# rcleuthold/awebox

Hardware: AMD Instinct MI355X
Metric: NLP f/g/Jacobian evals/sec, AP2 N=40 d=4 (higher is better)
Workload: dtype f64; 1 GPU; AP2 single kite, direct collocation radau N=40 d=4 zoh, 2048 NLP instances per step and GPU, one eval = f + g + grad f + J_g; n_v=6154, n_g=6103, nnz_jac=84726, batch_per_gpu=2048, parallelism=replicas x1

## Files before the change

### awebox_amd/csrc/awegpu.hip

```cpp
#include <hip/hip_runtime.h>

#include <algorithm>
#include <cmath>
#include <cstdio>
#include <cstdlib>
#include <cstring>
#include <memory>
#include <string>
#include <vector>

#include "../../include/awegpu.h"
#include "../../include/awegpu_rk4root.h"
#include "host_util.hpp"
#include "ap2_model.hpp"
#ifndef AWE_GEN_HEADER
#define AWE_GEN_HEADER "ap2_nodejac.gen.hpp"
#endif
#include AWE_GEN_HEADER
#include "ap2_tables.hpp"
#include "im_layout.hpp"

namespace {

using namespace awt;
using namespace hostu;




struct KArgs {
    const double* V;
    const double* P;
    const double* cst;
    DevColl coll;
    const ColorTabs* ct;
    const int* seg;
    const unsigned* glist;
    const int* glist_off;
    double* g;
    double* jac;
    double* grad;
    double* partial;
    double* f;
    int n_k, d, n_v, n_g, n_p, nnz, batch;
    int stride, rows, v_int0;
    int tang_total;
    int nscale;
    double kconst[kMaxConst];
    int nconst;
    int want_derivs;
    const double* nodebuf;
    int nb_stride;
    size_t tan_shoot, tan_radau;
    const double* objb;
    int ld;
    int grad_ld;
    int in_ld;
};

struct LaneIn {
    const double* w;
    unsigned long long seedA;
    unsigned int seedXD;
    double cxx;
    double tfs;
    __device__ __forceinline__ static double bit(unsigned long long m, int i) {
        return (double)(unsigned)((m >> i) & 1ull);
    }
    __device__ __forceinline__ awe::Dual operator()(int i) const {
        double t = bit(seedA, i);
        if (i >= AWE_NX && i < 2 * AWE_NX) {
            const int j = i - AWE_NX;
            if ((seedA >> j) & 1ull) t += cxx;
            if ((seedXD >> j) & 1u) t += 1.0;
            t += tfs * w[i];
        }
        return awe::Dual(w[i], t);
    }
};

struct NodeSink {
    double* tp;
    double* gv;
    double* dump;
    unsigned long long cm;
    bool c0;
    __device__ __forceinline__ void emit(int r, const awe::Dual& v) {
        double* ga = c0 ? gv + r : dump;
        *ga = v.v;
        const bool on = (cm >> r) & 1ull;
        double* ta = on ? tp + __popcll(cm & ((1ull << r) - 1ull)) : dump;
        *ta = v.d;
    }
    __device__ __forceinline__ void eq_row(int r, const awe::Dual& v) { emit(r, v); }
    __device__ __forceinline__ void ineq_row(int r, const awe::Dual& v) { emit(AWE_N_EQ + r, v); }
    __device__ __forceinline__ void power(const awe::Dual& v) { emit(kRowPower, v); }
    __device__ __forceinline__ void beta(const awe::Dual& v) { emit(kRowBeta, v); }
};


constexpr int kPreDirs = 7;
__device__ __forceinline__ int pre_var(int j) { return j < 6 ? j : kDirDiam; }

struct LdsSubmodels {
    const double* pr;
    unsigned long long seedA;
    __device__ __forceinline__ void kite_atmosphere(const awe::Dual&, const double*, awe::Dual& uw,
                                                    awe::Dual& rho) const {
        const double sd = ((seedA >> 2) & 1ull) ? 1.0 : 0.0;
        uw = awe::Dual(pr[24], sd * pr[25]);
        rho = awe::Dual(pr[26], sd * pr[27]);
    }
    __device__ __forceinline__ void tether_drag(const awe::Dual*, const awe::Dual*, const awe::Dual&,
                                                const double*, const double*, awe::Dual D[3]) const {
#pragma unroll
        for (int i = 0; i < 3; ++i) {
            double t = 0.0;
#pragma unroll
            for (int j = 0; j < kPreDirs; ++j)
                if ((seedA >> pre_var(j)) & 1ull) t += pr[3 + 3 * j + i];
            D[i] = awe::Dual(pr[i], t);
        }
    }
};

__device__ __forceinline__ double wave_sum(double v) {
#pragma unroll
    for (int off = 32; off > 0; off >>= 1) v += __shfl_xor(v, off);
    return v;
}

template <int D>
constexpr int waves_for() { return (D + 2) / 2; }

template <int D>
constexpr int nloc_pad() {
    return ((9 + AWE_NX + AWE_NU + AWE_NX + AWE_NZ + D * (AWE_NX + AWE_NZ) + AWE_NX) + 1) & ~1;
}

constexpr int kPstCost = 64, kPstThRef = 84, kPstRef = 86;
template <int D>
constexpr int pst_pad() {
    return (kPstRef + AWE_NX + AWE_NU + AWE_NX + AWE_NZ + D * (AWE_NX + AWE_NZ) + 1) & ~1;
}

template <int D>
constexpr int lds_fixed_doubles() {
    return nloc_pad<D>() + pst_pad<D>() + (D + 1) * (64 + kGvalStride + 64 + kPreStride) + ((D + 2) & ~1) + 64 + 2;
}


template <int D, int NT>
__device__ __forceinline__ void node_values_pass(const double* vloc, const double* C, int n_k, double* wn,
                                                 int tid) {
    constexpr int NN = D + 1;
    const double* vt = vloc;
    const double* vx = vloc + 9;
    const double* vu = vx + AWE_NX;
    const double* vxd = vu + AWE_NU;
    const double* vz = vxd + AWE_NX;
    const double* vcoll = vz + AWE_NZ;
// ... 599 lines not shown
    for (int i = tid; i < a.nscale; i += NT) {
        double sv = 1.0;
        if (i >= 1 && i <= NN * NN) sv = C[i - 1] * inv_h_tf;
        else if (i > NN * NN) sv = a.kconst[i - 1 - NN * NN];
        scl[i] = sv;
    }
    node_values_pass<D, NT>(vloc, C, a.n_k, wn, tid);
    if (tid == 0) tl[a.tang_total] = 1.0;

    const double* pcost = pst + kPstCost;
    const double* pw8 = pst;
    const double psi = vt[2 + kPhiPsi];
    const double w_track = pcost[kCostTracking] / a.cst[AWE_C_NORM_TRACKING];
    const double w_xdot = pcost[kCostXdotRegularisation] / a.cst[AWE_C_NORM_XDOT_REG];
    const double w_ureg = pcost[kCostURegularisation] / a.cst[AWE_C_NORM_U_REG];
    const double w_fict = pcost[kCostFictitious] / a.cst[AWE_C_NORM_FICTITIOUS];
    const double w_theta = pcost[kCostThetaRegularisation] / a.cst[AWE_C_NORM_THETA_REG];
    for (int n = 1 + wave; n < NN; n += W) {
        const int dir = lane;
        const int j = n - 1;
        const double wj = a.coll.w[j];
        const double* w = wn + n * 64;
        const double* rb = pst + kPstRef;
        const double* rcx = rb + 2 * AWE_NX + AWE_NU + AWE_NZ + j * (AWE_NX + AWE_NZ);
        const double* ru = rb + AWE_NX;
        const double cxx = C[n * NN + n] * inv_h_tf;
        double trk = 0.0, xdr = 0.0, oth = 0.0, dfd = 0.0;
        if (dir < AWE_NX) {
            const double e = w[dir] - rcx[dir], ww = pw8[dir] * w_track;
            const double xdv = w[AWE_NX + dir], wx = pw8[AWE_NX + dir] * w_xdot;
            trk = ww * (e * e);
            dfd = wj * (psi * (2.0 * ww * e) + cxx * (2.0 * wx * xdv));
        } else if (dir < 2 * AWE_NX) {
            const double xdv = w[dir], wx = pw8[dir] * w_xdot;
            xdr = wx * (xdv * xdv);
            dfd = wj * (2.0 * wx * xdv);
        } else if (dir < 2 * AWE_NX + AWE_NU) {
            const int i = dir - 2 * AWE_NX;
            const double e = w[dir] - ru[i], wu = pw8[dir] * (i < 6 ? w_fict : w_ureg);
            oth = wu * (e * e);
            dfd = wj * (2.0 * wu * e);
        } else if (dir == kDirZ) {
            const double e = w[dir] - rcx[AWE_NX], ww = pw8[dir] * w_track;
            trk = ww * (e * e);
            dfd = wj * psi * (2.0 * ww * e);
        } else if (dir == kDirDiam) {
            const double e = w[dir] - pst[kPstThRef], wt = pw8[dir] * w_theta;
            oth = wt * (e * e);
            dfd = wj * (2.0 * wt * e);
        }
        trk = wave_sum(trk);
        xdr = wave_sum(xdr);
        oth = wave_sum(oth);
        const double* on = objn + j * kObjNode;
        const double bv = on[0], pv = on[1];
        const double cb = pcost[kCostBeta] * wj / a.cst[AWE_C_NORM_BETA];
        const double cp = -pcost[kCostPower] * wj / (double)a.n_k;
        if (dir == kDirTf) dfd = -2.0 * wj * xdr * inv_tf;
        if (dir == kDirPsi) dfd = wj * trk - cp * pv;
#pragma unroll
        for (int i = 0; i < awe_gen::kNDbp; ++i)
            if (dir == awe_gen::kDbpDir[i]) dfd += on[2 + i];
        dfl[n * 64 + dir] = dfd;
        if (dir == 0) fnode[n] = wj * (psi * trk + xdr + oth) + cb * (bv * bv) + (1.0 - psi) * (cp * pv);
    }
    __syncthreads();

    const DevColl* cc = &a.coll;
    for (int i = tid; i < AWE_NX; i += NT) {
        double xf = 0.0;
#pragma unroll
        for (int rr = 0; rr < NN; ++rr) {
            if (cc->D[rr] == 0.0) continue;
            const double Xr = (rr == 0) ? vx[i] : vcoll[(rr - 1) * (AWE_NX + AWE_NZ) + i];
            xf += cc->D[rr] * Xr;
        }
        g[k * a.rows + AWE_N_EQ + AWE_N_INEQ + D * AWE_N_EQ + i] = vx1[i] - xf;
    }
    double* part = a.partial + ((size_t)b * a.n_k + k) * kNPartial;
    if (tid == 0) {
        double s = 0.0;
        for (int n = 1; n < NN; ++n) s += fnode[n];
        part[0] = s;
    }
    if (tid >= 1 && tid <= 3) {
        const int dcol = tid == 1 ? kDirDiam : (tid == 2 ? kDirTf : kDirPsi);
        double s = 0.0;
        for (int n = 1; n < NN; ++n) s += dfl[n * 64 + dcol];
        part[tid] = s;
    }
    for (int col = tid; col < a.stride; col += NT) {
        double gsum = 0.0;
        if (col < AWE_NX) {
#pragma unroll
            for (int n = 1; n < NN; ++n) gsum += C[n] * inv_h_tf * dfl[n * 64 + AWE_NX + col];
        } else if (col < AWE_NX + AWE_NU) {
            const int i = col - AWE_NX;
#pragma unroll
            for (int n = 1; n < NN; ++n) gsum += dfl[n * 64 + 2 * AWE_NX + i];
        } else if (col >= 2 * AWE_NX + AWE_NU + AWE_NZ) {
            const int q = col - (2 * AWE_NX + AWE_NU + AWE_NZ);
            const int r = 1 + q / (AWE_NX + AWE_NZ), e = q % (AWE_NX + AWE_NZ);
            if (e < AWE_NX) {
                gsum = dfl[r * 64 + e];
#pragma unroll
                for (int n = 1; n < NN; ++n)
                    if (n != r) gsum += C[r * NN + n] * inv_h_tf * dfl[n * 64 + AWE_NX + e];
            } else {
                gsum = dfl[r * 64 + kDirZ];
            }
        }
        grad[base + col] = gsum;
    }
    int g0s[kSegs], los[kSegs];
#pragma unroll
    for (int q = 0; q < kSegs; ++q) { g0s[q] = sg[3 * q]; los[q] = sg[3 * q + 2]; }
#pragma unroll
    for (int u = 0; u < kGatherPerThread; ++u) {
        const int i = tid + u * NT;
        if (i < total) {
            int g0 = g0s[0], lo = los[0];
#pragma unroll
            for (int q = 1; q < kSegs; ++q)
                if (i >= los[q]) { g0 = g0s[q]; lo = los[q]; }
            jac[g0 + i - lo] = scl[ge[u] >> 16] * tl[ge[u] & 0xffffu];
        }
    }
}

constexpr int kSoaMinBatch = 128;

using SoaSlots = im::SlotTraits<awe_gen::kTanIdx, awe_gen::kNTan, AWE_NX, 512>;
inline bool soa_xdot_slot(int kind, int slot) {
    static const im::SlotTab<SoaSlots> st2(2);
    return kind == 1 && st2.cnt[1][slot] == 2;
}
template <int KIND>
struct SoaJSink1 {
    double* jac;
    unsigned lb;
    const unsigned* dt;
    const double* xs;
    struct Ref {
        const SoaJSink1* s;
        int slot;
        __device__ __forceinline__ void operator=(double v) const { s->put(slot, v); }
    };
    __device__ __forceinline__ Ref operator[](int slot) const { return Ref{this, slot}; }
    __device__ __forceinline__ void put(int slot, double v) const {
        const bool xd = KIND == 1 && im::kSlots<SoaSlots, 2>.cnt[1][slot] == 2;
        __builtin_nontemporal_store(xd ? xs[0] * v : v, &im::at_byte(jac, dt[im::kSlots<SoaSlots, 1>.first[KIND][slot]] + lb));
    }
};
template <int D, int KIND>
using SoaJSink = std::conditional_t<D == 1, SoaJSink1<KIND>, im::JSink<SoaSlots, D, KIND>>;

struct SoaNodeArgs {
    DevColl coll;
    int n_k, batch, ld, n_v, n_g, n_p, stride, v_int0, rows, nib, total, dstride;
    unsigned ldj8;
    unsigned gld8;
    double kconst[kMaxConst];
};

__global__ __launch_bounds__(256) void ap2_soa_in_kernel(const double* __restrict__ V, const double* __restrict__ P,
                                                         double* __restrict__ VT, double* __restrict__ PT,
                                                         int batch, int n_v, int n_p, int ld) {
    im::transpose_in<true>(V, P, VT, PT, batch, n_v, n_p, ld);
}

__global__ __launch_bounds__(256) void soa_to_aos_kernel(const double* __restrict__ src, size_t ld,
                                                         double* __restrict__ dst, int batch, int n) {
    __shared__ double tile[64][65];
    const int i0 = blockIdx.x * 64, b0 = blockIdx.y * 64;
    const int tid = threadIdx.x;
    double r[16];
#pragma unroll
    for (int it = 0; it < 16; ++it) {
        const int e = tid + it * 256, il = e >> 6, bl = e & 63;
        r[it] = src[(size_t)min(i0 + il, n - 1) * ld + min(b0 + bl, batch - 1)];
    }
#pragma unroll
    for (int it = 0; it < 16; ++it) {
        const int e = tid + it * 256;
        tile[e >> 6][e & 63] = r[it];
    }
    __syncthreads();
#pragma unroll
    for (int it = 0; it < 16; ++it) {
        const int e = tid + it * 256, bl = e >> 6, il = e & 63;
        if (i0 + il < n && b0 + bl < batch)
            __builtin_nontemporal_store(tile[il][bl], &dst[(size_t)(b0 + bl) * n + i0 + il]);
    }
}

__global__ __launch_bounds__(256) void aos_to_soa_kernel(const double* __restrict__ src, double* __restrict__ dst,
                                                         size_t ld, int batch, int n) {
    __shared__ double tile[64][65];
    const int i0 = blockIdx.x * 64, b0 = blockIdx.y * 64;
    const int tid = threadIdx.x;
    double r[16];
#pragma unroll
    for (int it = 0; it < 16; ++it) {
        const int e = tid + it * 256, bl = e >> 6, il = e & 63;
        r[it] = src[(size_t)min(b0 + bl, batch - 1) * n + min(i0 + il, n - 1)];
    }
#pragma unroll
    for (int it = 0; it < 16; ++it) {
        const int e = tid + it * 256;
        tile[e >> 6][e & 63] = r[it];
    }
    __syncthreads();
#pragma unroll
    for (int it = 0; it < 16; ++it) {
        const int e = tid + it * 256, il = e >> 6, bl = e & 63;
        if (i0 + il < n && b0 + bl < batch) dst[(size_t)(i0 + il) * ld + b0 + bl] = tile[bl][il];
    }
}

#ifndef AWE_SOA_WAVES_PER_EU
#define AWE_SOA_WAVES_PER_EU 1
#endif

constexpr int kSoaG = awe_gen::kNThUsed;
constexpr int kSoaGlob = 6;
constexpr int kSoaCO = 2 * AWE_NX + AWE_NU + AWE_NZ;
constexpr int kSoaShootWaves = 3;
template <int D>
constexpr int soa_radau_waves() { return D < 4 ? D : 4; }
template <int D>
constexpr int soa_radau_rows() { return kSoaG + kSoaGlob + kSoaCO + D * (AWE_NX + AWE_NZ); }
constexpr int soa_shoot_rows() { return kSoaG + kSoaGlob + kSoaShootWaves * kSoaCO; }

struct SoaThUsed {
    short idx[awe_gen::kNThUsed > 0 ? awe_gen::kNThUsed : 1];
    constexpr SoaThUsed() : idx() {
        for (int i = 0; i < AWE_NTHETA0; ++i)
            if (awe_gen::kThRow[i] >= 0) idx[awe_gen::kThRow[i]] = (short)i;
    }
};
constexpr SoaThUsed kSoaThUsed{};
constexpr bool soa_th_used_ok() {
    int named[awe_gen::kNThUsed > 0 ? awe_gen::kNThUsed : 1] = {};
    for (int i = 0; i < AWE_NTHETA0; ++i) {
        const int r = awe_gen::kThRow[i];
        if (r >= awe_gen::kNThUsed) return false;
        if (r >= 0) ++named[r];
    }
    for (int r = 0; r < awe_gen::kNThUsed; ++r) {
        const int i = kSoaThUsed.idx[r];
        if (named[r] != 1 || i < 0 || i >= AWE_NTHETA0 || awe_gen::kThRow[i] != r) return false;
    }
    return true;
}
static_assert(soa_th_used_ok(), "kSoaThUsed is not the inverse of kThRow over the rows [0, kSoaG)");

struct SoaLdsTh {
    const double* l;
    __device__ __forceinline__ double operator[](int i) const { return l[awe_gen::kThRow[i] * 64]; }
};

__device__ __forceinline__ unsigned soa_glob_src(int q, unsigned& which) {
    which = q < 4 ? 0u : 1u;
    return q == 0 ? 1u : q == 1 ? 0u : q == 2 ? (unsigned)(AWE_NTH + kPhiGamma)
         : q == 3 ? (unsigned)(AWE_NTH + kPhiPsi) : q == 4 ? (unsigned)kCostBeta : (unsigned)kCostPower;
}

template <int I>
struct SoaWaveC { static constexpr int value = I; };
template <int W, int WV = 0, class F>
__device__ __forceinline__ void soa_per_wave(int wave, const F& f) {
    if constexpr (WV + 1 < W) {
        if (wave != WV) return soa_per_wave<W, WV + 1>(wave, f);
    }
    f(SoaWaveC<WV>{});
}

template <int NT, int U>
struct SoaOffsetLoads {
    unsigned r[U];
    template <class Src>
    __device__ __forceinline__ void issue(int n, int tid, const Src& src) {
#pragma unroll
        for (int u = 0; u < U; ++u) r[u] = *src(tid + u * NT < n ? tid + u * NT : n - 1);
    }
    __device__ __forceinline__ void commit(unsigned* dst, int n, unsigned row8, int tid) const {
#pragma unroll
        for (int u = 0; u < U; ++u)
            if (tid + u * NT < n) dst[tid + u * NT] = r[u] * row8;
    }
};

template <int W, int NROWS, int NTAB, class RowOf, class TabSrc>
__device__ __forceinline__ void soa_stage(double* lds, unsigned* ldt, int tid, int wave, int ib, int nact,
                                          const double* VT, const double* THT, unsigned ld8, unsigned row8,
                                          const RowOf& row_of, const TabSrc& tab_src) {
    constexpr int NT = 64 * W, UT = (NTAB + NT - 1) / NT;
    const int lane = tid & 63;
    const unsigned lb = 8u * (unsigned)(ib * 64 + (lane < nact ? lane : 0));
    double* lw = lds + lane;
    soa_per_wave<W>(wave, [&](auto wc) {
        constexpr int WV = decltype(wc)::value;
        constexpr int J = (NROWS - WV + W - 1) / W;
        constexpr int NF = (J + UT + 62) / 63, F = (J + UT + NF - 1) / NF;
        static_assert(F <= 63 && J > (NF - 1) * F, "a flight of more loads than vmcnt counts");
        auto load = [&](int r) {
            unsigned which;
            const unsigned row = row_of(r, which);
            return im::at(which ? THT : VT, row, ld8, lb);
        };
        SoaOffsetLoads<NT, UT> tab;
#pragma unroll
        for (int f = 0; f < NF; ++f) {
            double v[F];
#pragma unroll
            for (int j = f * F; j < J && j < (f + 1) * F; ++j) v[j - f * F] = load(WV + j * W);
            if (f == NF - 1) tab.issue(NTAB, tid, tab_src);
#pragma unroll
            for (int j = f * F; j < J && j < (f + 1) * F; ++j) lw[(WV + j * W) * 64] = v[j - f * F];
        }
        tab.commit(ldt, NTAB, row8, tid);
    });
}

struct SoaLdsShootIn {
    const double* l;
    int base;
    __device__ __forceinline__ double at(int r) const { return l[r * 64]; }
    __device__ __forceinline__ double operator()(int i) const {
        if (i < AWE_NX) return at(base + i);
        if (i < 2 * AWE_NX) return at(base + AWE_NX + AWE_NU + (i - AWE_NX));
        if (i < 2 * AWE_NX + AWE_NU) return at(base + AWE_NX + (i - 2 * AWE_NX));
        if (i < 2 * AWE_NX + AWE_NU + AWE_NZ) return at(base + 2 * AWE_NX + AWE_NU);
        if (i < AWE_NW) return at(kSoaG + (i == 2 * AWE_NX + AWE_NU + AWE_NZ ? 1 : 0));
        return at(kSoaG + 2);
    }
};

template <int D>
struct SoaLdsRadauIn {
    const double* l;
    int n;
    double inv_h_tf;
    const double* C;
    __device__ __forceinline__ double at(int r) const { return l[r * 64]; }
    __device__ __forceinline__ double operator()(int i) const {
        constexpr int NN = D + 1;
        constexpr int S0 = kSoaG + kSoaGlob;
        const int xc = S0 + kSoaCO + (n - 1) * (AWE_NX + AWE_NZ);
        if (i < AWE_NX) return at(xc + i);
        if (i < 2 * AWE_NX) {
            const int s = i - AWE_NX;
            double xp = C[n] * at(S0 + s);
#pragma unroll
            for (int r = 1; r < NN; ++r) xp += C[r * NN + n] * at(S0 + kSoaCO + (r - 1) * (AWE_NX + AWE_NZ) + s);
            return xp * inv_h_tf;
        }
        if (i < 2 * AWE_NX + AWE_NU) return at(S0 + AWE_NX + (i - 2 * AWE_NX));
        if (i < 2 * AWE_NX + AWE_NU + AWE_NZ) return at(xc + AWE_NX);
        if (i < AWE_NW) return at(kSoaG + (i == 2 * AWE_NX + AWE_NU + AWE_NZ ? 1 : 0));
        return at(kSoaG + 2);
    }
};

template <int D>
constexpr int soa_eval_waves() { return soa_radau_waves<D>() > kSoaShootWaves ? soa_radau_waves<D>() : kSoaShootWaves; }

template <int D>
__device__ __forceinline__ void soa_shoot_role(int t, double* lds, unsigned* ldt, const double* VT, const double* THT,
                                               const double* cst, const unsigned* dtab, const unsigned* ctab,
                                               const int* coff, double* g, double* jac, const SoaNodeArgs& a) {
    constexpr int NN = D + 1;
    constexpr int T0 = im::kSlots<SoaSlots, D>.total[0];
    const int nk3 = (a.n_k + kSoaShootWaves - 1) / kSoaShootWaves;
    const int ib = t / nk3, k0 = (t - ib * nk3) * kSoaShootWaves;
    const int tid = threadIdx.x, lane = tid & 63;
    const int wave = __builtin_amdgcn_readfirstlane(tid >> 6);
    const int nact = min(64, a.batch - ib * 64);
    const unsigned ld8 = 8u * a.ld;
    soa_stage<soa_eval_waves<D>(), soa_shoot_rows(), kSoaShootWaves * T0>(lds, ldt, tid, wave, ib, nact, VT, THT, ld8,
                                                                          a.ldj8,
        [&](int r, unsigned& which) -> unsigned {
            if (r < kSoaG) { which = 1; return AWE_NCOST + kSoaThUsed.idx[r]; }
            if (r < kSoaG + kSoaGlob) return soa_glob_src(r - kSoaG, which);
            which = 0;
            const int w = (r - kSoaG - kSoaGlob) / kSoaCO, c = r - kSoaG - kSoaGlob - w * kSoaCO;
            const int k = min(k0 + w, a.n_k - 1);
            return (unsigned)(a.v_int0 + k * a.stride + c);
        },
        [&](int i) {
            const int w = i / T0;
            return dtab + (size_t)(min(k0 + w, a.n_k - 1) * NN) * a.dstride + (i - w * T0);
        });
    __syncthreads();
    const int k = k0 + wave;
    if (wave >= kSoaShootWaves || k >= a.n_k || lane >= nact) return;
    const int b = ib * 64 + lane;
    const unsigned lb = 8u * b;
    const double* l = lds + lane;
    SoaLdsShootIn in{l, kSoaG + kSoaGlob + wave * kSoaCO};
    SoaLdsTh th{l};
    SoaJSink<D, 0> js{jac, lb, ldt + wave * T0, nullptr};
    awe_gen::ap2_node_shoot<1>(in, th, cst, g + (size_t)b * a.n_g + (size_t)k * a.rows, js);
    for (int q = coff[k]; q < coff[k + 1]; ++q) {
        const unsigned e = ctab[q];
        __builtin_nontemporal_store(a.kconst[e >> 24], &im::at(jac, e & 0xffffffu, a.ldj8, lb));
    }
}

constexpr int kSoaS0 = kSoaG + kSoaGlob;
constexpr int kSoaDead = kSoaS0 + AWE_NX + AWE_NU;
constexpr int kSoaIntWaves = 4;
template <int D>
constexpr int soa_radau_early() { return D - soa_radau_waves<D>(); }
template <int D>
constexpr int soa_radau_pool() { return awe_gen::kNDbp * soa_radau_waves<D>() + kSoaIntWaves * 3 * D; }
template <int D>
constexpr int soa_radau_extra() { return soa_radau_pool<D>() > kSoaS0 ? soa_radau_pool<D>() - kSoaS0 : 0; }
template <int D>
__device__ __forceinline__ constexpr int soa_pool_row(int p) {
    return p < kSoaS0 ? p : soa_radau_rows<D>() + (p - kSoaS0);
}
template <int D>
__device__ __forceinline__ constexpr int soa_obj_row(int j, int e) {
    constexpr int E = soa_radau_early<D>();
    if (e < 2) return kSoaDead + 2 * j + e;
    if (j < E) return kSoaDead + 2 * D + awe_gen::kNDbp * j + (e - 2);
    return awe_gen::kNDbp * (j - E) + (e - 2);
}
template <int D>
__device__ __forceinline__ constexpr int soa_red_row(int v, int c, int n) {
    return soa_pool_row<D>(awe_gen::kNDbp * soa_radau_waves<D>() + (v * 3 + c) * D + n);
}

struct SoaLdsRef {
    double* l;
    int r0;
    __device__ __forceinline__ double& operator[](int i) const { return l[(r0 + i) * 64]; }
};

constexpr int kSoaRadauBarriers = 4;
template <int D>
__device__ __forceinline__ void soa_radau_role(int t, double* lds, unsigned* ldt, const double* VT, const double* PT,
                                               const double* cst, const unsigned* dtab, double* g, double* jac,
                                               double* grad, double* partial, const SoaNodeArgs& a) {
    constexpr int NN = D + 1;
    constexpr int CO = kSoaCO;
    constexpr int W = soa_radau_waves<D>();
    constexpr int T1 = im::kSlots<SoaSlots, D>.total[1];
    constexpr int E = soa_radau_early<D>();
    constexpr int VW = kSoaIntWaves;
    constexpr int NV = (VW + W - 1) / W;
    constexpr int NS = (AWE_NX + VW - 1) / VW;
    constexpr int NSU = (AWE_NU + VW - 1) / VW;
    static_assert(E >= 0 && E <= W, "a wavefront runs at most two Radau nodes");
    static_assert(2 * D + awe_gen::kNDbp * E <= AWE_NX + AWE_NZ, "objective rows beyond the slice's unread rows");
    static_assert(awe_gen::kNDbp * W <= kSoaS0, "dbp rows beyond the pool");
    constexpr int BW = soa_eval_waves<D>();
    const int ib = t / a.n_k, k = t % a.n_k;
    const int tid = threadIdx.x, lane = tid & 63;
    const int wave = __builtin_amdgcn_readfirstlane(tid >> 6);
    const int nact = min(64, a.batch - ib * 64);
    const unsigned ld8 = 8u * a.ld;
    const int c0 = a.v_int0 + k * a.stride;
    const double* THT = PT + (size_t)(a.n_v + AWE_NW) * a.ld;
    soa_stage<BW, soa_radau_rows<D>(), D * T1>(lds, ldt, tid, wave, ib, nact, VT, THT, ld8, a.ldj8,
        [&](int r, unsigned& which) -> unsigned {
            if (r < kSoaG) { which = 1; return AWE_NCOST + kSoaThUsed.idx[r]; }
            if (r < kSoaG + kSoaGlob) return soa_glob_src(r - kSoaG, which);
            which = 0;
            return (unsigned)(c0 + (r - kSoaG - kSoaGlob));
        },
        [&](int i) {
            const int j = i / T1;
            return dtab + (size_t)(k * NN + 1 + j) * a.dstride + (i - j * T1);
        });
    __syncthreads();
    if constexpr (BW > W) {
        if (wave >= W) {
#pragma unroll
            for (int s = 1; s < kSoaRadauBarriers; ++s) __syncthreads();
            return;
        }
    }
    const bool act = lane < nact;
    const int b = ib * 64 + lane;
    const int bb = act ? b : ib * 64;
    const unsigned lb = 8u * bb;
    double* lw = lds + lane;
    const double* l = lw;
    const double tf = l[kSoaG * 64];
    const double h = 1.0 / a.n_k;
    const double inv_h_tf = 1.0 / h / tf;
    const double psi = l[(kSoaG + 3) * 64];
    double dq[awe_gen::kNDbp];
#pragma unroll
    for (int q = 0; q < awe_gen::kNDbp; ++q) dq[q] = 0.0;
    if (act) {
        SoaLdsTh th{l};
        for (int n = 1 + wave; n < NN; n += W) {
            const int j = n - 1;
            const double wj = a.coll.w[j];
            const double cb = l[(kSoaG + 4) * 64] * wj / cst[AWE_C_NORM_BETA];
            const double cp = -l[(kSoaG + 5) * 64] * wj / (double)a.n_k;
            SoaLdsRadauIn<D> in{l, n, inv_h_tf, a.coll.C};
            double xs[D];
#pragma unroll
            for (int q = 0; q < D; ++q) xs[q] = a.coll.C[(q < n ? q : q + 1) * NN + n] * inv_h_tf;
            SoaJSink<D, 1> js{jac, lb, ldt + (n - 1) * T1, xs};
            SoaLdsRef ob{lw, kSoaDead + 2 * j};
            awe_gen::ap2_node_radau<1>(in, a.coll.C[n * NN + n] * inv_h_tf, 1.0 / tf, cb, (1.0 - psi) * cp, th, cst,
                                       g + (size_t)b * a.n_g + (size_t)k * a.rows + AWE_N_EQ + AWE_N_INEQ + j * AWE_N_EQ,
                                       js, dq, ob);
            if constexpr (E > 0) {
                if (j < E) {
#pragma unroll
                    for (int q = 0; q < awe_gen::kNDbp; ++q)
                        lw[(kSoaDead + 2 * D + awe_gen::kNDbp * j + q) * 64] = dq[q];
                }
            }
        }
    }

    auto Pp = [&](int col) { return im::at(PT, (unsigned)col, ld8, lb); };
    const int wo = a.n_v;
    const int co = a.n_v + AWE_NW;
    const double inv_tf = 1.0 / tf;
    const double diam = l[(kSoaG + 1) * 64];
    const double cbeta = l[(kSoaG + 4) * 64], cpower = l[(kSoaG + 5) * 64];
    const double w_track = Pp(co + kCostTracking) / cst[AWE_C_NORM_TRACKING];
    const double w_xdot = Pp(co + kCostXdotRegularisation) / cst[AWE_C_NORM_XDOT_REG];
    const double w_ureg = Pp(co + kCostURegularisation) / cst[AWE_C_NORM_U_REG];
    const double w_fict = Pp(co + kCostFictitious) / cst[AWE_C_NORM_FICTITIOUS];
    const double w_theta = Pp(co + kCostThetaRegularisation) / cst[AWE_C_NORM_THETA_REG];
    const double* C = a.coll.C;
    double pxn[NV][NS], pwt[NV][NS], pwx[NV][NS], pref[NV][NS][D], puref[NV][NSU], puw[NV][NSU];
#pragma unroll
    for (int vi = 0; vi < NV; ++vi) {
        const int v = wave + vi * W;
#pragma unroll
        for (int s = 0; s < NS; ++s) {
            const int i = v + s * VW;
            const bool on = v < VW && i < AWE_NX;
            const int ii = on ? i : 0;
            pxn[vi][s] = im::at(VT, (unsigned)(c0 + a.stride + ii), ld8, lb);
            pwt[vi][s] = Pp(wo + ii);
            pwx[vi][s] = Pp(wo + AWE_NX + ii);
#pragma unroll
            for (int j = 0; j < D; ++j) pref[vi][s][j] = Pp(c0 + CO + j * (AWE_NX + AWE_NZ) + ii);
        }
#pragma unroll
        for (int s = 0; s < NSU; ++s) {
            const int i = v + s * VW;
            const int ii = v < VW && i < AWE_NU ? i : 0;
            puref[vi][s] = Pp(c0 + AWE_NX + ii);
            puw[vi][s] = Pp(wo + 2 * AWE_NX + ii);
        }
    }
    const double pdiam = Pp(0), pwdiam = Pp(wo + kDirDiam), pwz = Pp(wo + kDirZ);
    double pzref[D];
#pragma unroll
    for (int j = 0; j < D; ++j) pzref[j] = Pp(c0 + CO + j * (AWE_NX + AWE_NZ) + AWE_NX);
    __syncthreads();
    {
        const int jf = wave + W * ((D - 1 - wave) / W) - E;
#pragma unroll
        for (int q = 0; q < awe_gen::kNDbp; ++q) lw[(awe_gen::kNDbp * jf + q) * 64] = dq[q];
    }
    __syncthreads();
    auto X = [&](int r, int i) { return l[(r == 0 ? kSoaS0 + i : kSoaS0 + CO + (r - 1) * (AWE_NX + AWE_NZ) + i) * 64]; };
    auto ob = [&](int j, int e) { return l[soa_obj_row<D>(j, e) * 64]; };
    struct GRef { double* p; __device__ void operator=(double v) const { __builtin_nontemporal_store(v, p); } };
    auto GR = [&](int col) { return GRef{&im::at(grad, (unsigned)(c0 + col), a.gld8, lb)}; };
    double* gc = g + (size_t)bb * a.n_g + (size_t)k * a.rows + AWE_N_EQ + AWE_N_INEQ + D * AWE_N_EQ;
#pragma unroll
    for (int vi = 0; vi < NV; ++vi) {
        const int v = wave + vi * W;
        if (v >= VW) break;
        double trk[D], xdr[D], oth[D];
#pragma unroll
        for (int n = 0; n < D; ++n) trk[n] = xdr[n] = oth[n] = 0.0;
#pragma unroll
        for (int s = 0; s < NS; ++s) {
            const int i = v + s * VW;
            if (i >= AWE_NX) break;
            double Xr[NN];
#pragma unroll
            for (int r = 0; r < NN; ++r) Xr[r] = X(r, i);
            const double wtr = pwt[vi][s] * w_track, wx = pwx[vi][s] * w_xdot;
            double dx[NN], dxd[NN];
#pragma unroll
            for (int n = 1; n < NN; ++n) {
                const int j = n - 1;
                const double wj = a.coll.w[j];
                double xp = C[n] * Xr[0];
#pragma unroll
                for (int r = 1; r < NN; ++r) xp += C[r * NN + n] * Xr[r];
                const double xdv = xp * inv_h_tf;
                const double cxx = C[n * NN + n] * inv_h_tf;
                const double e = Xr[n] - pref[vi][s][j];
                trk[j] += wtr * (e * e);
                xdr[j] += wx * (xdv * xdv);
                double d = wj * (psi * (2.0 * wtr * e) + cxx * (2.0 * wx * xdv));
#pragma unroll
                for (int q = 0; q < awe_gen::kNDbp; ++q)
                    if (i == awe_gen::kDbpDir[q]) d += ob(j, 2 + q);
                dx[n] = d;
                dxd[n] = wj * (2.0 * wx * xdv);
            }
            double xf = 0.0;
#pragma unroll
            for (int rr = 0; rr < NN; ++rr) {
                if (a.coll.D[rr] == 0.0) continue;
                xf += a.coll.D[rr] * Xr[rr];
            }
            const double xnext = pxn[vi][s];
            if (act) {
                double gs = 0.0;
#pragma unroll
                for (int n = 1; n < NN; ++n) gs += C[n] * inv_h_tf * dxd[n];
                GR(i) = gs;
#pragma unroll
                for (int r = 1; r < NN; ++r) {
                    double sr = dx[r];
#pragma unroll
                    for (int n = 1; n < NN; ++n)
                        if (n != r) sr += C[r * NN + n] * inv_h_tf * dxd[n];
                    GR(CO + (r - 1) * (AWE_NX + AWE_NZ) + i) = sr;
                }
                gc[i] = xnext - xf;
            }
        }
#pragma unroll
        for (int s = 0; s < NSU; ++s) {
            const int i = v + s * VW;
            if (i >= AWE_NU) break;
            const double e = l[(kSoaS0 + AWE_NX + i) * 64] - puref[vi][s];
            const double wu = puw[vi][s] * (i < 6 ? w_fict : w_ureg);
            double gs = 0.0;
#pragma unroll
            for (int n = 1; n < NN; ++n) {
                oth[n - 1] += wu * (e * e);
                gs += a.coll.w[n - 1] * (2.0 * wu * e);
            }
            if (act) GR(AWE_NX + i) = gs;
        }
        for (int i = v; i < AWE_NX + AWE_NZ; i += VW)
            if (act) GR(AWE_NX + AWE_NU + i) = 0.0;
#pragma unroll
        for (int n = 0; n < D; ++n) {
            lw[soa_red_row<D>(v, 0, n) * 64] = trk[n];
            lw[soa_red_row<D>(v, 1, n) * 64] = xdr[n];
            lw[soa_red_row<D>(v, 2, n) * 64] = oth[n];
        }
    }
    __syncthreads();
    if (wave != 0) return;
    const double ed = diam - pdiam, wt = pwdiam * w_theta;
    const double wz = pwz * w_track;
    double fsum = 0.0, sdiam = 0.0, stf = 0.0, spsi = 0.0;
#pragma unroll
    for (int n = 1; n < NN; ++n) {
        const int j = n - 1;
        const double wj = a.coll.w[j];
        double tr = 0.0, xd = 0.0, ot = 0.0;
#pragma unroll
        for (int w = 0; w < VW; ++w) {
            tr += l[soa_red_row<D>(w, 0, j) * 64];
            xd += l[soa_red_row<D>(w, 1, j) * 64];
            ot += l[soa_red_row<D>(w, 2, j) * 64];
        }
        const double ez = l[(kSoaS0 + CO + j * (AWE_NX + AWE_NZ) + AWE_NX) * 64] - pzref[j];
        tr += wz * (ez * ez);
        double dz = wj * psi * (2.0 * wz * ez);
#pragma unroll
        for (int q = 0; q < awe_gen::kNDbp; ++q)
            if (kDirZ == awe_gen::kDbpDir[q]) dz += ob(j, 2 + q);
        if (act) GR(CO + j * (AWE_NX + AWE_NZ) + AWE_NX) = dz;
        ot += wt * (ed * ed);
        const double bv = ob(j, 0), pv = ob(j, 1);
        const double cb = cbeta * wj / cst[AWE_C_NORM_BETA];
        const double cp = -cpower * wj / (double)a.n_k;
        double dd = wj * (2.0 * wt * ed), dt_ = -2.0 * wj * xd * inv_tf, dp = wj * tr - cp * pv;
#pragma unroll
        for (int q = 0; q < awe_gen::kNDbp; ++q) {
            if (kDirDiam == awe_gen::kDbpDir[q]) dd += ob(j, 2 + q);
            if (kDirTf == awe_gen::kDbpDir[q]) dt_ += ob(j, 2 + q);
            if (kDirPsi == awe_gen::kDbpDir[q]) dp += ob(j, 2 + q);
        }
        fsum += wj * (psi * tr + xd + ot) + cb * (bv * bv) + (1.0 - psi) * (cp * pv);
        sdiam += dd;
        stf += dt_;
        spsi += dp;
    }
    if (!act) return;
    double* part = partial + ((size_t)b * a.n_k + k) * kNPartial;
    part[0] = fsum;
    part[1] = sdiam;
    part[2] = stf;
    part[3] = spsi;
}

#ifndef AWE_SOA_SHOOT_FIRST
#define AWE_SOA_SHOOT_FIRST 0
#endif

__device__ __forceinline__ int soa_xcd_tile(int bx, int total) {
    const int per = (total + 7) / 8;
    return (bx & 7) * per + (bx >> 3);
}

template <int D>
__global__ __launch_bounds__(64 * soa_eval_waves<D>()) __attribute__((amdgpu_waves_per_eu(AWE_SOA_WAVES_PER_EU)))
void ap2_soa_eval_kernel(const double* __restrict__ VT, const double* __restrict__ PT,
                         const double* __restrict__ cst, const unsigned* __restrict__ dtab,
                         const unsigned* __restrict__ ctab, const int* __restrict__ coff,
                         double* __restrict__ g, double* __restrict__ jac, double* __restrict__ grad,
                         double* __restrict__ partial, SoaNodeArgs a) {
    constexpr int T0 = im::kSlots<SoaSlots, D>.total[0], T1 = im::kSlots<SoaSlots, D>.total[1];
    constexpr int RR = soa_radau_rows<D>() + soa_radau_extra<D>();
    constexpr int ROWS = RR > soa_shoot_rows() ? RR : soa_shoot_rows();
    constexpr int NTAB = D * T1 > kSoaShootWaves * T0 ? D * T1 : kSoaShootWaves * T0;
    static_assert(ROWS * 512 + NTAB * 4 <= 160 * 1024, "LDS image too large");
    __shared__ double buf[ROWS * 64 + (NTAB + 1) / 2];
    double* lds = buf;
    unsigned* ldt = reinterpret_cast<unsigned*>(buf + ROWS * 64);
    const int nr = a.nib * a.n_k;
    const int ns = a.nib * ((a.n_k + kSoaShootWaves - 1) / kSoaShootWaves);
    const int first = AWE_SOA_SHOOT_FIRST ? im::xcd_grid(ns) : im::xcd_grid(nr);
    const bool low = (int)blockIdx.x < first;
    const int bx = low ? (int)blockIdx.x : (int)blockIdx.x - first;
    if (low != (bool)AWE_SOA_SHOOT_FIRST) {
        const int t = soa_xcd_tile(bx, nr);
        if (t >= nr) return;
        soa_radau_role<D>(t, lds, ldt, VT, PT, cst, dtab, g, jac, grad, partial, a);
    } else {
        const int t = soa_xcd_tile(bx, ns);
        if (t >= ns) return;
        soa_shoot_role<D>(t, lds, ldt, VT, PT + (size_t)(a.n_v + AWE_NW) * a.ld, cst, dtab, ctab, coff, g, jac, a);
    }
}

__global__ __launch_bounds__(64) void ap2_finalize_kernel(KArgs a) {
    const int lane = threadIdx.x;
    const int b = blockIdx.x;
    const size_t vs = a.in_ld ? (size_t)a.in_ld : 1;
    const double* Vb = a.in_ld ? a.V + b : a.V + (size_t)b * a.n_v;
    const double* Pb = a.in_ld ? a.P + b : a.P + (size_t)b * a.n_p;
    auto V = [&](int i) { return Vb[(size_t)i * vs]; };
    auto cost = [&](int i) { return Pb[(size_t)(a.n_v + AWE_NW + i) * vs]; };
    double* g = a.g + (size_t)b * a.n_g;
    auto grad_at = [&](int i) -> double& {
        return a.grad_ld ? a.grad[(size_t)i * a.grad_ld + b] : a.grad[(size_t)b * a.n_v + i];
    };
    const double* part = a.partial + (size_t)b * a.n_k * kNPartial;

    double s[kNPartial] = {0.0, 0.0, 0.0, 0.0};
    for (int k = lane; k < a.n_k; k += 64)
        for (int c = 0; c < kNPartial; ++c) s[c] += part[k * kNPartial + c];
    for (int off = 32; off > 0; off >>= 1)
        for (int c = 0; c < kNPartial; ++c) s[c] += __shfl_xor(s[c], off);

    const double tf = V(1), tf_ref = Pb[vs];
    const int last = a.v_int0 + (a.n_k - 1) * a.stride + 2 * AWE_NX + AWE_NU + AWE_NZ +
                     (a.d - 1) * (AWE_NX + AWE_NZ);
    if (lane < AWE_NX) {
        const int i = kPeriodicOrder[lane];
        g[a.n_k * a.rows + lane] = V(a.v_int0 + i) - V(last + i);
    }
    constexpr int phi_cost_map[AWE_NPHI] = {3, 6, 4, 5, 7, 8, 9};
    if (lane == 0) {
        double fh = 0.0;
        for (int i = 0; i < AWE_NPHI; ++i) fh += cost(phi_cost_map[i]) * V(AWE_NTH + i);
        const double time_cost = cost(kCostTf) * (tf - tf_ref) * (tf - tf_ref);
        a.f[b] = s[0] + time_cost + fh;
    }
    if (a.want_derivs) {
        if (lane == 0) grad_at(0) = s[1];
        if (lane == 1) grad_at(1) = s[2] + cost(kCostTf) * 2.0 * (tf - tf_ref);
        if (lane >= 2 && lane < 2 + AWE_NPHI) {
            const int i = lane - 2;
            double gphi = cost(phi_cost_map[i]);
            if (i == kPhiPsi) gphi += s[3];
            grad_at(AWE_NTH + i) = gphi;
        }
        if (lane >= 2 + AWE_NPHI && lane < 2 + AWE_NPHI + AWE_NXI) grad_at(lane) = 0.0;
        if (lane < AWE_NX) grad_at(a.v_int0 + a.n_k * a.stride + lane) = 0.0;
    }
}



struct ValueIn {
    const double* w;
    __device__ __forceinline__ double operator()(int i) const { return w[i]; }
};

struct ValueSink {
    double* gv;
    __device__ __forceinline__ void eq_row(int r, double v) { gv[r] = v; }
    __device__ __forceinline__ void ineq_row(int r, double v) { gv[AWE_N_EQ + r] = v; }
    __device__ __forceinline__ void power(double v) { gv[kRowPower] = v; }
    __device__ __forceinline__ void beta(double v) { gv[kRowBeta] = v; }
};

template <int D>
__global__ __launch_bounds__(64) void ap2_value_kernel(KArgs a) {
    constexpr int NN = D + 1;
    const int tid = threadIdx.x;
    const int k = blockIdx.x % a.n_k;
    const int b = blockIdx.x / a.n_k;
    const double* V = a.V + (size_t)b * a.n_v;
    const double* P = a.P + (size_t)b * a.n_p;
    const double* th = P + a.n_v + AWE_NW + AWE_NCOST;
    const double* cost = P + a.n_v + AWE_NW;
    const double* wts = P + a.n_v;
    const double* vref = P;
    double* g = a.g + (size_t)b * a.n_g;
    const double* C = a.coll.C;
    __shared__ double vloc[nloc_pad<D>()];
    __shared__ double wn[NN * 64];
    __shared__ double gval[NN * kGvalStride];
    __shared__ double fnode[NN + 1];
    const int base = a.v_int0 + k * a.stride;
    for (int i = tid; i < 9; i += 64) vloc[i] = V[i];
    for (int i = tid; i < a.stride + AWE_NX; i += 64) vloc[9 + i] = V[base + i];
    __syncthreads();
    node_values_pass<D, 64>(vloc, C, a.n_k, wn, tid);
    const double* vt = vloc;
    const double* vx = vloc + 9;
    const double* vcoll = vx + AWE_NX + AWE_NU + AWE_NX + AWE_NZ;
    const double* vx1 = vcoll + D * (AWE_NX + AWE_NZ);
    if (tid < NN) {
        const int n = tid;
        ValueIn in{wn + n * 64};
        ValueSink sink{gval + n * kGvalStride};
        awe::ap2_node<double>(in, vt[2 + kPhiGamma], th, a.cst, sink, n == 0, awe::InlineSubmodels());
        double fn = 0.0;
        if (n > 0) {
            const int j = n - 1;
            const double wj = a.coll.w[j];
            const double* w = wn + n * 64;
            const double* rb = vref + base;
            const double* rcx = rb + 2 * AWE_NX + AWE_NU + AWE_NZ + j * (AWE_NX + AWE_NZ);
            const double* ru = rb + AWE_NX;
            const double psi = vt[2 + kPhiPsi];
            const double w_track = cost[kCostTracking] / a.cst[AWE_C_NORM_TRACKING];
            const double w_xdot = cost[kCostXdotRegularisation] / a.cst[AWE_C_NORM_XDOT_REG];
            const double w_ureg = cost[kCostURegularisation] / a.cst[AWE_C_NORM_U_REG];
            const double w_fict = cost[kCostFictitious] / a.cst[AWE_C_NORM_FICTITIOUS];
            const double w_theta = cost[kCostThetaRegularisation] / a.cst[AWE_C_NORM_THETA_REG];
            double trk = 0.0, xdr = 0.0, oth = 0.0;
            for (int i = 0; i < AWE_NX; ++i) {
                const double e = w[i] - rcx[i];
                trk += wts[i] * w_track * (e * e);
                const double xdv = w[AWE_NX + i];
                xdr += wts[AWE_NX + i] * w_xdot * (xdv * xdv);
            }
            for (int i = 0; i < AWE_NU; ++i) {
                const double e = w[2 * AWE_NX + i] - ru[i];
                oth += wts[2 * AWE_NX + i] * (i < 6 ? w_fict : w_ureg) * (e * e);
            }
            {
                const double e = w[kDirZ] - rcx[AWE_NX];
                trk += wts[kDirZ] * w_track * (e * e);
                const double et = w[kDirDiam] - vref[0];
                oth += wts[kDirDiam] * w_theta * (et * et);
            }
            const double bv = gval[n * kGvalStride + kRowBeta];
            const double pv = gval[n * kGvalStride + kRowPower];
            const double cb = cost[kCostBeta] * wj / a.cst[AWE_C_NORM_BETA];
            const double cp = -cost[kCostPower] * wj / (double)a.n_k;
            fn = wj * (psi * trk + xdr + oth) + cb * (bv * bv) + (1.0 - psi) * (cp * pv);
        }
        fnode[n] = fn;
// ... 1722 lines not shown
```

Baseline: 5.236 million evals/s.

## Hold Jacobian destination offset tables in wave registers instead of LDS

For collocation degrees 2-4, each wavefront now loads its node's Jacobian destination offset table into vector registers (one entry per lane) and fetches entries via readlane, instead of staging all tables into shared memory. This removes the LDS table region and the LDS reads in the sink. Inactive lanes now run the node code against a clamped batch index so the whole wave stays convergent. The cost is more VGPR pressure and extra readlane instructions per Jacobian store, and the node loop assumes one node per wave.

```diff
diff --git a/awebox_amd/csrc/awegpu.hip b/awebox_amd/csrc/awegpu.hip
--- a/awebox_amd/csrc/awegpu.hip
+++ b/awebox_amd/csrc/awegpu.hip
@@ -7,6 +7,7 @@
 #include <cstring>
 #include <memory>
 #include <string>
+#include <utility>
 #include <vector>
 
 #include "../../include/awegpu.h"
@@ -912,8 +913,54 @@
         __builtin_nontemporal_store(xd ? xs[0] * v : v, &im::at_byte(jac, dt[im::kSlots<SoaSlots, 1>.first[KIND][slot]] + lb));
     }
 };
+template <int D>
+constexpr bool soa_lane_table() { return D >= 2 && D <= 4; }
 template <int D, int KIND>
-using SoaJSink = std::conditional_t<D == 1, SoaJSink1<KIND>, im::JSink<SoaSlots, D, KIND>>;
+constexpr int soa_lane_regs() { return (im::kSlots<SoaSlots, D>.total[KIND] + 63) / 64; }
+template <int D, int KIND>
+constexpr bool soa_lane_slots_ok() {
+    for (int s = 0; s < SoaSlots::kNTan[KIND]; ++s) {
+        const int f = im::kSlots<SoaSlots, D>.first[KIND][s], c = im::kSlots<SoaSlots, D>.cnt[KIND][s];
+        if (f < 0 || c < 1 || f + c > 64 * soa_lane_regs<D, KIND>()) return false;
+    }
+    return true;
+}
+template <int D, int KIND>
+struct SoaLaneSink {
+    static constexpr int NVT = soa_lane_regs<D, KIND>();
+    static_assert(soa_lane_slots_ok<D, KIND>(), "a slot's destinations beyond the table registers");
+    double* jac;
+    unsigned lb;
+    int tv[NVT];
+    const double* xs;
+    struct Ref {
+        const SoaLaneSink* s;
+        int slot;
+        __device__ __forceinline__ void operator=(double v) const { s->put(slot, v); }
+    };
+    __device__ __forceinline__ Ref operator[](int slot) const { return Ref{this, slot}; }
+    __device__ __forceinline__ void store(int i, double v) const {
+        const unsigned off = (unsigned)__builtin_amdgcn_readlane(tv[i >> 6], i & 63);
+        char* row = reinterpret_cast<char*>(jac) + (size_t)off;
+        __builtin_nontemporal_store(v, reinterpret_cast<double*>(row + (size_t)lb));
+    }
+    __device__ __forceinline__ void put(int slot, double v) const {
+        const int f = im::kSlots<SoaSlots, D>.first[KIND][slot], c = im::kSlots<SoaSlots, D>.cnt[KIND][slot];
+        if (c == 1) {
+            store(f, v);
+            return;
+        }
+        put_xdot(f, v, std::make_integer_sequence<int, D>{});
+    }
+    template <int... Q>
+    __device__ __forceinline__ void put_xdot(int f, double v, std::integer_sequence<int, Q...>) const {
+        (store(f + Q, xs[Q] * v), ...);
+    }
+};
+template <int D, int KIND>
+using SoaJSink = std::conditional_t<D == 1, SoaJSink1<KIND>,
+                                    std::conditional_t<soa_lane_table<D>(), SoaLaneSink<D, KIND>,
+                                                       im::JSink<SoaSlots, D, KIND>>>;
 
 struct SoaNodeArgs {
     DevColl coll;
@@ -1051,17 +1098,67 @@
     }
 };
 
-template <int W, int NROWS, int NTAB, class RowOf, class TabSrc>
-__device__ __forceinline__ void soa_stage(double* lds, unsigned* ldt, int tid, int wave, int ib, int nact,
-                                          const double* VT, const double* THT, unsigned ld8, unsigned row8,
-                                          const RowOf& row_of, const TabSrc& tab_src) {
-    constexpr int NT = 64 * W, UT = (NTAB + NT - 1) / NT;
+template <int NT, int NTAB, class Src>
+struct SoaLdsTab {
+    static constexpr int U = (NTAB + NT - 1) / NT;
+    unsigned* ldt;
+    unsigned row8;
+    const Src& src;
+    SoaOffsetLoads<NT, U> r;
+    template <int WV>
+    static constexpr int loads() { return U; }
+    template <int WV>
+    __device__ __forceinline__ void issue(int tid) { r.issue(NTAB, tid, src); }
+    template <int WV>
+    __device__ __forceinline__ void commit(int tid) const { r.commit(ldt, NTAB, row8, tid); }
+};
+template <int T, int NODEW>
+struct SoaLaneTab {
+    static constexpr int NVT = (T + 63) / 64;
+    const unsigned* row;
+    unsigned row8;
+    int tv[NVT];
+    template <int WV>
+    static constexpr int loads() { return WV < NODEW ? NVT : 0; }
+    template <int WV>
+    __device__ __forceinline__ void issue(int tid) {
+        if constexpr (WV < NODEW) {
+            const int lane = tid & 63;
+#pragma unroll
+            for (int j = 0; j < NVT; ++j) tv[j] = (int)row[64 * j + lane < T ? 64 * j + lane : T - 1];
+        }
+    }
+    template <int WV>
+    __device__ __forceinline__ void commit(int) {
+        if constexpr (WV < NODEW) {
+#pragma unroll
+            for (int j = 0; j < NVT; ++j) tv[j] = (int)((unsigned)tv[j] * row8);
+        }
+    }
+};
+template <int D, int KIND, class Tab>
+__device__ __forceinline__ SoaJSink<D, KIND> soa_sink(const Tab& tab, double* jac, unsigned lb, const unsigned* dt,
+                                                      const double* xs) {
+    if constexpr (soa_lane_table<D>()) {
+        SoaJSink<D, KIND> s{jac, lb, {}, xs};
+#pragma unroll
+        for (int j = 0; j < Tab::NVT; ++j) s.tv[j] = tab.tv[j];
+        return s;
+    } else {
+        return SoaJSink<D, KIND>{jac, lb, dt, xs};
+    }
+}
+
+template <int W, int NROWS, class Tab, class RowOf>
+__device__ __forceinline__ void soa_stage(double* lds, Tab& tab, int tid, int wave, int ib, int nact,
+                                          const double* VT, const double* THT, unsigned ld8, const RowOf& row_of) {
     const int lane = tid & 63;
     const unsigned lb = 8u * (unsigned)(ib * 64 + (lane < nact ? lane : 0));
     double* lw = lds + lane;
     soa_per_wave<W>(wave, [&](auto wc) {
         constexpr int WV = decltype(wc)::value;
         constexpr int J = (NROWS - WV + W - 1) / W;
+        constexpr int UT = Tab::template loads<WV>();
         constexpr int NF = (J + UT + 62) / 63, F = (J + UT + NF - 1) / NF;
         static_assert(F <= 63 && J > (NF - 1) * F, "a flight of more loads than vmcnt counts");
         auto load = [&](int r) {
@@ -1069,17 +1166,16 @@
             const unsigned row = row_of(r, which);
             return im::at(which ? THT : VT, row, ld8, lb);
         };
-        SoaOffsetLoads<NT, UT> tab;
 #pragma unroll
         for (int f = 0; f < NF; ++f) {
             double v[F];
 #pragma unroll
             for (int j = f * F; j < J && j < (f + 1) * F; ++j) v[j - f * F] = load(WV + j * W);
-            if (f == NF - 1) tab.issue(NTAB, tid, tab_src);
+            if (f == NF - 1) tab.template issue<WV>(tid);
 #pragma unroll
             for (int j = f * F; j < J && j < (f + 1) * F; ++j) lw[(WV + j * W) * 64] = v[j - f * F];
         }
-        tab.commit(ldt, NTAB, row8, tid);
+        tab.template commit<WV>(tid);
     });
 }
 
@@ -1138,29 +1234,33 @@
     const int wave = __builtin_amdgcn_readfirstlane(tid >> 6);
     const int nact = min(64, a.batch - ib * 64);
     const unsigned ld8 = 8u * a.ld;
-    soa_stage<soa_eval_waves<D>(), soa_shoot_rows(), kSoaShootWaves * T0>(lds, ldt, tid, wave, ib, nact, VT, THT, ld8,
-                                                                          a.ldj8,
-        [&](int r, unsigned& which) -> unsigned {
-            if (r < kSoaG) { which = 1; return AWE_NCOST + kSoaThUsed.idx[r]; }
-            if (r < kSoaG + kSoaGlob) return soa_glob_src(r - kSoaG, which);
-            which = 0;
-            const int w = (r - kSoaG - kSoaGlob) / kSoaCO, c = r - kSoaG - kSoaGlob - w * kSoaCO;
-            const int k = min(k0 + w, a.n_k - 1);
-            return (unsigned)(a.v_int0 + k * a.stride + c);
-        },
-        [&](int i) {
-            const int w = i / T0;
-            return dtab + (size_t)(min(k0 + w, a.n_k - 1) * NN) * a.dstride + (i - w * T0);
-        });
+    auto row_of = [&](int r, unsigned& which) -> unsigned {
+        if (r < kSoaG) { which = 1; return AWE_NCOST + kSoaThUsed.idx[r]; }
+        if (r < kSoaG + kSoaGlob) return soa_glob_src(r - kSoaG, which);
+        which = 0;
+        const int w = (r - kSoaG - kSoaGlob) / kSoaCO, c = r - kSoaG - kSoaGlob - w * kSoaCO;
+        const int k = min(k0 + w, a.n_k - 1);
+        return (unsigned)(a.v_int0 + k * a.stride + c);
+    };
+    auto tab_row = [&](int w) { return dtab + (size_t)(min(k0 + w, a.n_k - 1) * NN) * a.dstride; };
+    auto tab_src = [&](int i) { return tab_row(i / T0) + i % T0; };
+    using LdsTab = SoaLdsTab<64 * soa_eval_waves<D>(), kSoaShootWaves * T0, decltype(tab_src)>;
+    using Tab = std::conditional_t<soa_lane_table<D>(), SoaLaneTab<T0, kSoaShootWaves>, LdsTab>;
+    Tab tab = [&] {
+        if constexpr (soa_lane_table<D>()) return Tab{tab_row(wave), a.ldj8, {}};
+        else return Tab{ldt, a.ldj8, tab_src, {}};
+    }();
+    soa_stage<soa_eval_waves<D>(), soa_shoot_rows()>(lds, tab, tid, wave, ib, nact, VT, THT, ld8, row_of);
     __syncthreads();
     const int k = k0 + wave;
-    if (wave >= kSoaShootWaves || k >= a.n_k || lane >= nact) return;
-    const int b = ib * 64 + lane;
+    if (wave >= kSoaShootWaves || k >= a.n_k) return;
+    if (!soa_lane_table<D>() && lane >= nact) return;
+    const int b = ib * 64 + (lane < nact ? lane : 0);
     const unsigned lb = 8u * b;
     const double* l = lds + lane;
     SoaLdsShootIn in{l, kSoaG + kSoaGlob + wave * kSoaCO};
     SoaLdsTh th{l};
-    SoaJSink<D, 0> js{jac, lb, ldt + wave * T0, nullptr};
+    const SoaJSink<D, 0> js = soa_sink<D, 0>(tab, jac, lb, soa_lane_table<D>() ? nullptr : ldt + wave * T0, nullptr);
     awe_gen::ap2_node_shoot<1>(in, th, cst, g + (size_t)b * a.n_g + (size_t)k * a.rows, js);
     for (int q = coff[k]; q < coff[k + 1]; ++q) {
         const unsigned e = ctab[q];
@@ -1224,17 +1324,21 @@
     const unsigned ld8 = 8u * a.ld;
     const int c0 = a.v_int0 + k * a.stride;
     const double* THT = PT + (size_t)(a.n_v + AWE_NW) * a.ld;
-    soa_stage<BW, soa_radau_rows<D>(), D * T1>(lds, ldt, tid, wave, ib, nact, VT, THT, ld8, a.ldj8,
-        [&](int r, unsigned& which) -> unsigned {
-            if (r < kSoaG) { which = 1; return AWE_NCOST + kSoaThUsed.idx[r]; }
-            if (r < kSoaG + kSoaGlob) return soa_glob_src(r - kSoaG, which);
-            which = 0;
-            return (unsigned)(c0 + (r - kSoaG - kSoaGlob));
-        },
-        [&](int i) {
-            const int j = i / T1;
-            return dtab + (size_t)(k * NN + 1 + j) * a.dstride + (i - j * T1);
-        });
+    auto row_of = [&](int r, unsigned& which) -> unsigned {
+        if (r < kSoaG) { which = 1; return AWE_NCOST + kSoaThUsed.idx[r]; }
+        if (r < kSoaG + kSoaGlob) return soa_glob_src(r - kSoaG, which);
+        which = 0;
+        return (unsigned)(c0 + (r - kSoaG - kSoaGlob));
+    };
+    auto tab_row = [&](int j) { return dtab + (size_t)(k * NN + 1 + j) * a.dstride; };
+    auto tab_src = [&](int i) { return tab_row(i / T1) + i % T1; };
+    static_assert(!soa_lane_table<D>() || E == 0, "a wavefront's table registers hold one node's row");
+    using Tab = std::conditional_t<soa_lane_table<D>(), SoaLaneTab<T1, W>, SoaLdsTab<64 * BW, D * T1, decltype(tab_src)>>;
+    Tab tab = [&] {
+        if constexpr (soa_lane_table<D>()) return Tab{tab_row(wave), a.ldj8, {}};
+        else return Tab{ldt, a.ldj8, tab_src, {}};
+    }();
+    soa_stage<BW, soa_radau_rows<D>()>(lds, tab, tid, wave, ib, nact, VT, THT, ld8, row_of);
     __syncthreads();
     if constexpr (BW > W) {
         if (wave >= W) {
@@ -1256,9 +1360,9 @@
     double dq[awe_gen::kNDbp];
 #pragma unroll
     for (int q = 0; q < awe_gen::kNDbp; ++q) dq[q] = 0.0;
-    if (act) {
+    if (soa_lane_table<D>() || act) {
         SoaLdsTh th{l};
-        for (int n = 1 + wave; n < NN; n += W) {
+        auto node = [&](int n) {
             const int j = n - 1;
             const double wj = a.coll.w[j];
             const double cb = l[(kSoaG + 4) * 64] * wj / cst[AWE_C_NORM_BETA];
@@ -1267,10 +1371,10 @@
             double xs[D];
 #pragma unroll
             for (int q = 0; q < D; ++q) xs[q] = a.coll.C[(q < n ? q : q + 1) * NN + n] * inv_h_tf;
-            SoaJSink<D, 1> js{jac, lb, ldt + (n - 1) * T1, xs};
+            const SoaJSink<D, 1> js = soa_sink<D, 1>(tab, jac, lb, soa_lane_table<D>() ? nullptr : ldt + (n - 1) * T1, xs);
             SoaLdsRef ob{lw, kSoaDead + 2 * j};
             awe_gen::ap2_node_radau<1>(in, a.coll.C[n * NN + n] * inv_h_tf, 1.0 / tf, cb, (1.0 - psi) * cp, th, cst,
-                                       g + (size_t)b * a.n_g + (size_t)k * a.rows + AWE_N_EQ + AWE_N_INEQ + j * AWE_N_EQ,
+                                       g + (size_t)bb * a.n_g + (size_t)k * a.rows + AWE_N_EQ + AWE_N_INEQ + j * AWE_N_EQ,
                                        js, dq, ob);
             if constexpr (E > 0) {
                 if (j < E) {
@@ -1279,6 +1383,11 @@
                         lw[(kSoaDead + 2 * D + awe_gen::kNDbp * j + q) * 64] = dq[q];
                 }
             }
+        };
+        if constexpr (soa_lane_table<D>()) {
+            node(1 + wave);
+        } else {
+            for (int n = 1 + wave; n < NN; n += W) node(n);
         }
     }
 
@@ -1480,7 +1589,7 @@
     constexpr int T0 = im::kSlots<SoaSlots, D>.total[0], T1 = im::kSlots<SoaSlots, D>.total[1];
     constexpr int RR = soa_radau_rows<D>() + soa_radau_extra<D>();
     constexpr int ROWS = RR > soa_shoot_rows() ? RR : soa_shoot_rows();
-    constexpr int NTAB = D * T1 > kSoaShootWaves * T0 ? D * T1 : kSoaShootWaves * T0;
+    constexpr int NTAB = soa_lane_table<D>() ? 0 : D * T1 > kSoaShootWaves * T0 ? D * T1 : kSoaShootWaves * T0;
     static_assert(ROWS * 512 + NTAB * 4 <= 160 * 1024, "LDS image too large");
     __shared__ double buf[ROWS * 64 + (NTAB + 1) / 2];
     double* lds = buf;
```

Result: no change. 5.230 million evals/s, median of 3 (-0.1%).
